# bdsaglam/torch-scae

Measured on AMD Instinct MI355X. Metric: images/sec SCAE fwd+bwd, MNIST 40x40 bs=128, 1/2/4/8 MI355X, higher is better.
Workload: dtype f32

## Files before the change

### include/scae_hip.h

```cpp
#ifndef SCAE_HIP_H
#define SCAE_HIP_H

#include <stdint.h>

#ifdef __cplusplus
extern "C" {
#endif

#define SCAE_ABI_VERSION 3

#define SCAE_OK 0
#define SCAE_ERR_BAD_ARG (-1)
#define SCAE_ERR_UNSUPPORTED (-2)

#define SCAE_MAX_CHANNELS 4
#define SCAE_ATTN_MAX_SET 64
#define SCAE_RENDER_MAX_TEMPLATE_ELEMS 4096

int scae_abi_version(void);
const char *scae_error_string(int code);

void *scae_launch_list_begin(void *stream);
int scae_launch_list_end(void *list);
int scae_launch_list_size(const void *list);
// ... 607 lines not shown
    const float *cls_b, const int64_t *label, const scae_loss_extras *extras, float *out12,
    float *workspace, int B, int O, int M, int ncls, int n_classes_cfg, int prior_type,
    int post_type, int sparsity_on, const float *weights5, float within_const,
    const float *cp_caps_presence, const float *cp_posterior, const float *cp_w,
    const float *cp_bias, float *prior_prob, float *post_prob, int cp_B, int cp_O, int cp_M,
    int cp_ncls, const scae_scaled_sum *extra_sums, int n_extra, void *stream);
int scae_loss_tail_fwd_class_probs_sink_f32(
    const float *lpp, const float *posterior, const float *caps_presence, const float *cls_w,
    const float *cls_b, const int64_t *label, const scae_loss_extras *extras, float *out12,
    float *workspace, int B, int O, int M, int ncls, int n_classes_cfg, int prior_type,
    int post_type, int sparsity_on, const float *weights5, float within_const,
    const float *cp_caps_presence, const float *cp_posterior, const float *cp_w,
    const float *cp_bias, float *prior_prob, float *post_prob, int cp_B, int cp_O, int cp_M,
    int cp_ncls, const scae_scaled_sum *extra_sums, int n_extra, scae_eval_sink *sink,
    void *stream);
int scae_loss_tail_bwd_f32(const float *lpp, const float *posterior,
                           const float *caps_presence, const float *cls_w,
                           const float *cls_b, const int64_t *label,
                           const scae_loss_extras *extras, const float *gout12,
                           const float *workspace, float *g_lpp, float *g_posterior,
                           float *g_caps_presence, float *g_cls_w,
                           float *g_cls_b, int B, int O, int M, int ncls, int n_classes_cfg,
                           int prior_type, int post_type, int sparsity_on,
                           const float *weights5, float within_const, void *stream);

#define SCAE_EVAL_ACC_DOUBLES 17
int scae_eval_tail_f32(const float *lpp, const float *posterior, const float *caps_presence,
                       const float *cls_w, const float *cls_b, const int64_t *label,
                       const scae_loss_extras *extras, float *out12, float *workspace, int B,
                       int O, int M, int ncls, int n_classes_cfg, int prior_type,
// ... 146 lines not shown
```

### torch_scae_amd/_lib.py

```python
import ctypes
import os
from ctypes import (POINTER, Structure, c_char_p, c_double, c_float, c_int,
                    c_int64, c_uint32, c_uint64, c_void_p)

_HERE = os.path.dirname(os.path.abspath(__file__))
LIB_PATH = os.environ.get("SCAE_HIP_LIB") or os.path.join(_HERE, "lib",
                                                        "libscae_hip.so")

P = c_void_p


class DecoderDesc(Structure):
    _fields_ = [("templates", P), ("templates_alpha", P), ("pose", P),
                ("presence", P), ("bg_image", P), ("bg_value", P),
                ("bg_mixing_logit", P), ("temperature_logit", P),
                ("out_scale", P),
                ("B", c_int), ("M", c_int), ("C", c_int), ("th", c_int),
                ("tw", c_int), ("H", c_int), ("W", c_int),
                ("template_repeat", c_int)]


class LikelihoodBwdDesc(Structure):
    _fields_ = [(n, P) for n in (
        "vote", "scale", "vote_presence", "dummy_vote", "x", "presence",
# ... 286 lines not shown
                                  + [c_int] * 7 + [P],
    "scae_capsule_votes_bwd_f32": [P] * 8 + [c_float] + [P] * 11
                                  + [c_int] * 7 + [P],
    "scae_capsule_likelihood_fwd_f32": [P] * 17 + [c_int] * 3 + [P],
    "scae_capsule_likelihood_bwd_f32": [P] * 22 + [c_int] * 3 + [P],
    "scae_loss_tail_supported": [c_int] * 3,
    "scae_loss_tail_workspace_floats": [c_int] * 3,
    "scae_loss_tail_fwd_f32": [P] * 6 + [POINTER(LossExtras), P, P] + [c_int] * 8
    + [POINTER(c_float), c_float, P],
    "scae_loss_tail_defer_preferred": [c_int] * 2,
    "scae_loss_tail_combine_f32": [P] * 6 + [POINTER(LossExtras), P, P] + [c_int] * 8
    + [POINTER(c_float), c_float, P],
    "scae_loss_tail_fwd_class_probs_f32": [P] * 6 + [POINTER(LossExtras), P, P]
    + [c_int] * 8 + [POINTER(c_float), c_float] + [P] * 6 + [c_int] * 4
    + [POINTER(ScaledSum), c_int, P],
    "scae_loss_tail_bwd_f32": [P] * 6 + [POINTER(LossExtras)] + [P] * 7
    + [c_int] * 8 + [POINTER(c_float), c_float, P],
    "scae_eval_tail_f32": [P] * 6 + [POINTER(LossExtras), P, P] + [c_int] * 8
    + [POINTER(c_float), c_float] + [P] * 5,
    "scae_loss_tail_fwd_class_probs_sink_f32": [P] * 6 + [POINTER(LossExtras), P, P]
    + [c_int] * 8 + [POINTER(c_float), c_float] + [P] * 6 + [c_int] * 4
    + [POINTER(ScaledSum), c_int, P, P],
    "scae_eval_tail_sink_f32": [P] * 6 + [POINTER(LossExtras), P, P] + [c_int] * 8
    + [POINTER(c_float), c_float] + [P] * 6,
    "scae_eval_accumulate_f32": [P] * 5 + [c_int] * 2 + [P] * 3,
    "scae_train_log_f32": [P] * 3 + [POINTER(TrainLogDesc), c_int, P],
    "scae_eval_features_f32": [P, P, c_int, c_int, c_int, P, P],
    "scae_kmeans_supported": [c_int] * 2,
    "scae_kmeans_groups": [c_int64, c_int],
    "scae_kmeans_lloyd_f32": [POINTER(KMeansDesc), c_int, P],
# ... 121 lines not shown
```

### torch_scae_amd/csrc/capsule_likelihood_dev.h

```cpp
#pragma once
#include "common.h"

namespace scae_lk {
namespace {
constexpr int NT = 1024;
constexpr int OMAX = 64;
constexpr float kLog001 = -4.605170185988091f;

__device__ __forceinline__ float vote_lp(const float *vt, const float *xv, float sc) {
  const float inv2v = 1.f / (2.f * sc * sc), ls = logf(sc);
  float acc = 0.f;
#pragma unroll
  for (int i = 0; i < 6; ++i) {
    const float d = xv[i] - vt[i];
    acc += -(d * d) * inv2v - ls - scae::kHalfLog2Pi;
  }
  return acc;
}

template <int G>
__device__ __forceinline__ float group_sum(float v) {
  static_assert(G == 16, "one DPP row");
  return scae::row_sum16(v);
}
// ... 103 lines not shown
      }
    }
    sm = group_sum<16>(sm);
    sp = group_sum<16>(sp);
    if (m < M && l == 0) {
      s.max_ml[m] = mx_ml;
      s.lse_ml[m] = mx_ml + logf(sm);
      s.max_post[m] = mx_po;
      s.sum_post[m] = sp;
      s.win[m] = (float)win;
    }
  }
  __syncthreads();
}

template <bool BIG>
__global__ __launch_bounds__(1024) void likelihood_fwd_kernel(
    LkArgs a, float *__restrict__ lpp, float *__restrict__ binary, float *__restrict__ winner,
    float *__restrict__ winner_presence, int64_t *__restrict__ winner_idx,
    int64_t *__restrict__ is_from_capsule, float *__restrict__ soft_winner,
    float *__restrict__ soft_winner_presence, float *__restrict__ posterior,
    float *__restrict__ mixing_log_prob, float *__restrict__ mixing_logit) {
  extern __shared__ __attribute__((aligned(16))) float smem[];
  const int O = a.O, M = a.M, tid = threadIdx.x;
  const LkSmem s = lk_carve(smem, O, M);
  for (int b = blockIdx.x; b < a.B; b += gridDim.x) {
    __syncthreads();
    lk_stats<BIG, NT>(a, s, b);
    for (int e = tid; e < (O + 1) * M; e += NT) {
      const int o = e / M, m = e - o * M;
      const size_t g1 = (size_t)b * (O + 1) * M + e;
      const float ml = o < O ? s.ml[e] : kLog001;
      const float post = o < O ? s.post[e] : kLog001 + kLog001;
      const float pp = expf(post - s.max_post[m]) / s.sum_post[m];
      mixing_logit[g1] = ml;
      mixing_log_prob[g1] = ml - s.lse_ml[m];
      posterior[g1] = pp;
      if (o < O) {
        binary[(size_t)b * O * M + e] = ml > kLog001 ? 1.f : 0.f;
        s.ml[e] = pp;
      }
    }
    __syncthreads();
    for (int t = tid; t < ((M * 7 * 4 + NT - 1) / NT) * NT; t += NT) {
      const int e = t >> 2, part = t & 3;
      const bool pose = e < M * 6, live = e < M * 7;
      const int m = pose ? e / 6 : e - M * 6, i = pose ? e - m * 6 : 0;
      float acc = 0.f;
      if (live) {
        if (pose) {
#pragma unroll 6
          for (int o = part; o < O; o += 4)
            acc = fmaf(s.ml[o * M + m], a.vote[(((size_t)b * O + o) * M + m) * 6 + i], acc);
        } else {
#pragma unroll 6
          for (int o = part; o < O; o += 4)
            acc = fmaf(s.ml[o * M + m], a.vp[((size_t)b * O + o) * M + m], acc);
        }
      }
      acc += scae::xor1_f(acc);
      acc += scae::xor2_f(acc);
      if (!live || part != 0) continue;
      const size_t idx = (size_t)b * M + m;
      const int win = (int)s.win[m];
      if (pose) {
        const float ppd = expf(kLog001 + kLog001 - s.max_post[m]) / s.sum_post[m];
        soft_winner[idx * 6 + i] = fmaf(ppd, a.dummy_vote[m * 6 + i], acc);
        winner[idx * 6 + i] = a.vote[(((size_t)b * O + win) * M + m) * 6 + i];
      } else {
        const float lse_post = s.max_post[m] + logf(s.sum_post[m]);
        lpp[idx] = a.presence ? lse_post * a.presence[idx] : lse_post;
        soft_winner_presence[idx] = acc;
        winner_presence[idx] = a.vp[((size_t)b * O + win) * M + m];
        winner_idx[idx] = win;
        is_from_capsule[idx] = win / M;
      }
    }
  }
}

template <bool BIG, int NT>
__device__ __forceinline__ void likelihood_bwd_body(
    LkArgs a, const int64_t *__restrict__ winner_idx, const float *__restrict__ g_lpp,
    const float *__restrict__ g_winner, const float *__restrict__ g_winner_presence,
    const float *__restrict__ g_soft_winner, const float *__restrict__ g_soft_winner_presence,
    const float *__restrict__ g_posterior, const float *__restrict__ g_mlp,
    const float *__restrict__ g_mlogit, float *__restrict__ gvote, float *__restrict__ gscale,
    float *__restrict__ gvp, float *__restrict__ gx, float *__restrict__ gpresence,
    float *__restrict__ gdummy, float *smem, int blk, int nblk) {
  const int O = a.O, M = a.M, tid = threadIdx.x;
  const LkSmem s = lk_carve(smem, O, M);
  float *s_gpp = s.aux;
// ... 124 lines not shown
```

### torch_scae_amd/csrc/loss_tail.hip

```cpp
#include "class_probs_dev.h"
#include "common.h"
#include "loss_tail_dev.h"

namespace {
using namespace scae_tail;
constexpr int MAXCLS = 32;

__device__ __forceinline__ float ent_term_grad(float p, float k) {
  const float q = p * k;
  return q < scae::kLogSafeEps ? 1e8f : -(logf(q) + 1.f);
}

__device__ __forceinline__ float within_term(const float *x, float r, int O, int type,
                                             float cw, int lane) {
  if (type == 0) return (r - cw) * (r - cw);
  const float k = type == 2 ? (float)O : 1.f;
  float w = 0.f;
  for (int o = lane; o < O; o += NTI) w += ent_term(x[o] / (r + 1e-8f), k);
  return scae::wave_sum(w);
}

__device__ __forceinline__ float cls_xe(const TailArgs &a, const float *x, int label, int lane,
                                        float &gl) {
  const bool on = lane < a.ncls;
// ... 11 lines not shown
    z = (z0 + z1) + (z2 + z3);
  }
  const float mx = scae::wave_max(z);
  float p = on ? expf(z - mx) : 0.f;
  p /= scae::wave_sum(p);
  const float mx2 = scae::wave_max(on ? p : -INFINITY);
  const float q = on ? expf(p - mx2) : 0.f;
  const float sum2 = scae::wave_sum(q);
  const float plabel = scae::wave_sum(lane == label ? p : 0.f);
  const float dq = on ? q / sum2 - (lane == label ? 1.f : 0.f) : 0.f;
  const float dot = scae::wave_sum(p * dq);
  gl = p * (dq - dot);
  return mx2 + logf(sum2) - plabel;
}

__global__ __launch_bounds__(NTI) void tail_image_kernel(TailArgs a, Ws ws, scae_cp::Args cpa,
                                                        int n_cp) {
  extern __shared__ __attribute__((aligned(16))) float smem[];
  const int B = a.B, O = a.O, M = a.M, b = blockIdx.x, lane = threadIdx.x;
  if (b >= B) {
    __shared__ scae_cp::Lds s_cpl;
    scae_cp::body(cpa, s_cpl, b - B, lane);
    return;
  }
  float *s_cp = smem, *s_mass = smem + O, *s_raw = smem + 2 * O;
  float rc = 0.f, rm = 0.f;
  for (int o = lane; o < O; o += NTI) {
    const float xc = a.cp[(size_t)b * O + o];
    const float *pr = a.posterior + ((size_t)b * (O + 1) + o) * M;
    float t = 0.f;
    if ((M & 3) == 0) {
      const float4 *p4 = reinterpret_cast<const float4 *>(pr);
      for (int m = 0; m < M / 4; ++m) {
        const float4 v = p4[m];
        t += (v.x + v.y) + (v.z + v.w);
      }
    } else {
      for (int m = 0; m < M; ++m) t += pr[m];
    }
// ... 18 lines not shown
  float xe_c = 0.f, xe_m = 0.f;
  if (a.label) {
    const int label = (int)a.label[b];
    float g0, g1;
    xe_c = cls_xe(a, s_cp, label, lane, g0);
    xe_m = cls_xe(a, s_raw, label, lane, g1);
    if (lane < a.ncls) {
      ws.gl[((size_t)b * 2 + 0) * a.ncls + lane] = g0;
      ws.gl[((size_t)b * 2 + 1) * a.ncls + lane] = g1;
    }
  }
  if (lane == 0) {
    float *p = ws.part + (size_t)b * 8;
    p[0] = lp, p[1] = wc, p[2] = wm, p[3] = xe_c, p[4] = xe_m, p[5] = rc, p[6] = rm, p[7] = 0.f;
  }
}

template <int NTC>
__global__ __launch_bounds__(NTC) void tail_combine_kernel(TailArgs a, scae_loss_extras x, Ws ws,
                                                          float *out) {
  extern __shared__ __attribute__((aligned(16))) float smem[];
  combine_body<NTC>(a, x, ws, out, smem);
}

template <int NTC>
__global__ __launch_bounds__(NTC) void tail_combine_log_kernel(TailArgs a, scae_loss_extras x,
                                                              Ws ws, float *out,
                                                              TrainLogArgs g) {
  extern __shared__ __attribute__((aligned(16))) float smem[];
  combine_body<NTC>(a, x, ws, out, smem);
// ... 300 lines not shown
extern "C" int scae_loss_tail_fwd_class_probs_f32(
    const float *lpp, const float *posterior, const float *caps_presence, const float *cls_w,
    const float *cls_b, const int64_t *label, const scae_loss_extras *extras, float *out12,
    float *workspace, int B, int O, int M, int ncls, int n_classes_cfg, int prior_type,
    int post_type, int sparsity_on, const float *weights5, float within_const,
    const float *cp_caps_presence, const float *cp_posterior, const float *cp_w,
    const float *cp_bias, float *prior_prob, float *post_prob, int cp_B, int cp_O, int cp_M,
    int cp_ncls, const scae_scaled_sum *extra_sums, int n_extra, void *stream) {
  return scae_loss_tail_fwd_class_probs_sink_f32(
      lpp, posterior, caps_presence, cls_w, cls_b, label, extras, out12, workspace, B, O, M,
      ncls, n_classes_cfg, prior_type, post_type, sparsity_on, weights5, within_const,
      cp_caps_presence, cp_posterior, cp_w, cp_bias, prior_prob, post_prob, cp_B, cp_O, cp_M,
      cp_ncls, extra_sums, n_extra, nullptr, stream);
}

extern "C" int scae_loss_tail_bwd_f32(const float *lpp, const float *posterior,
                                      const float *caps_presence, const float *cls_w,
                                      const float *cls_b, const int64_t *label,
                                      const scae_loss_extras *extras, const float *gout12,
                                      const float *workspace, float *g_lpp, float *g_posterior,
                                      float *g_caps_presence, float *g_cls_w, float *g_cls_b,
                                      int B, int O, int M, int ncls, int n_classes_cfg,
                                      int prior_type, int post_type, int sparsity_on,
                                      const float *weights5, float within_const, void *stream) {
  TailArgs a;
  int rc = fill_tail(a, lpp, posterior, caps_presence, cls_w, cls_b, label, B, O, M, ncls,
                     n_classes_cfg, prior_type, post_type, sparsity_on, weights5, within_const);
  if (rc) return rc;
  SCAE_REQUIRE(g_lpp && g_posterior && g_caps_presence && workspace);
  if (!gout12 && !(extras && extras->g_loss)) return SCAE_ERR_BAD_ARG;
// ... 33 lines not shown
```

### torch_scae_amd/object_decoder.py

```python
import torch
import torch.nn as nn

from . import math_ops, ops
from .general_utils import AttrDict, prod
from .nn_ext import GroupedMLP
from .nn_utils import rand_like


class CapsuleLayer(nn.Module):

    n_transform_params = 6

    def __init__(self, n_caps, dim_feature, n_votes, dim_caps,
                 hidden_sizes=(128,), caps_dropout_rate=0.0,
                 learn_vote_scale=False, allow_deformations=True,
                 noise_type=None, noise_scale=0., similarity_transform=True):
        super().__init__()
        self.n_caps = n_caps
        self.dim_feature = dim_feature
        self.hidden_sizes = list(hidden_sizes)
        self.dim_caps = dim_caps
        self.caps_dropout_rate = caps_dropout_rate
        self.n_votes = n_votes
        self.learn_vote_scale = learn_vote_scale
# ... 130 lines not shown
        return AttrDict(vote=vote, scale=scale, vote_presence=vote_presence,
                        presence_logit_per_caps=logit_caps,
                        presence_logit_per_vote=logit_vote,
                        cpr_dynamic_reg_loss=reg)


class CapsuleLikelihood:

    def __init__(self, vote, scale, vote_presence, dummy_vote):
        self.n_caps = vote.shape[1]
        self.vote = vote
        self.scale = scale
        self.vote_presence = vote_presence
        self.dummy_vote = dummy_vote

    def __call__(self, x, presence=None, _extra_sums=(), _defer_sums=False):
        batch_size, n_input_points, dim_in = x.shape
        if dim_in != 6 or self.vote.shape[-1] != 6:
            raise ValueError("the capsule likelihood kernel is built for "
                             "6-dim poses")
        (lpp, binary, winner, winner_presence, _widx, is_from_capsule,
         soft_winner, soft_winner_presence, posterior, mixing_log_prob,
         mixing_logit, log_prob) = ops.capsule_likelihood(
            self.vote, self.scale, self.vote_presence, self.dummy_vote, x,
            presence.float() if presence is not None else None,
            defer_sum=True)
        sums = [(lpp.detach(), 1.0 / batch_size, log_prob.detach()),
                *_extra_sums]
        if not _defer_sums:
            ops.scaled_sums(sums)
        return AttrDict(
            **(dict(_pending_sums=sums) if _defer_sums else {}),
            _log_prob_per_point=lpp,
            _posterior_full=posterior,
            log_prob=log_prob,
            vote_presence_binary=binary,
            winner=winner,
            winner_presence=winner_presence,
            soft_winner=soft_winner,
            soft_winner_presence=soft_winner_presence,
            posterior_mixing_prob=posterior[:, :-1],
# ... 3 lines not shown
        )


class CapsuleObjectDecoder(nn.Module):
    def __init__(self, capsule_layer: CapsuleLayer):
        super().__init__()
        self.capsule_layer = capsule_layer
        self.dummy_vote = nn.Parameter(torch.zeros(
            1, 1, capsule_layer.n_votes, capsule_layer.n_transform_params))

    @property
    def n_obj_capsules(self):
        return self.capsule_layer.n_caps

    def forward(self, obj_encoding: torch.Tensor, part_pose: torch.Tensor,
                part_presence: torch.Tensor = None, _defer_sums=False):
        vote, scale, vote_presence, logit_caps, logit_vote, reg, \
            caps_presence, reg_partial = self.capsule_layer._votes(
                obj_encoding, defer_reg=True)
        res = AttrDict(vote=vote,
                       scale=scale, vote_presence=vote_presence,
                       presence_logit_per_caps=logit_caps,
                       presence_logit_per_vote=logit_vote,
                       cpr_dynamic_reg_loss=reg)
        res.caps_presence = caps_presence
        likelihood = CapsuleLikelihood(vote=res.vote, scale=res.scale,
                                       vote_presence=res.vote_presence,
                                       dummy_vote=self.dummy_vote)
        res.update(likelihood(part_pose, presence=part_presence, _extra_sums=[
            (reg_partial, 0.5 / obj_encoding.shape[0], reg.detach())],
            _defer_sums=_defer_sums))
        return res


def capsule_l2_loss(caps_presence, n_classes: int,
                    within_example_constant=None, **_ignored):
    n_examples, n_caps = caps_presence.shape
    row_target = n_caps / n_classes if within_example_constant is None \
        else within_example_constant
    col_target = n_examples / n_classes
    row_mass, col_mass = caps_presence.sum(1), caps_presence.sum(0)
    return ((row_mass - row_target).square().mean(),
            (col_mass - col_target).square().mean())


def _scaled_self_entropy(mass, dim, k):
# ... 21 lines not shown
```

### torch_scae_amd/ops.py

```python
import ctypes
import functools

import numpy as np
import torch

from . import _lib, step_plan
from ._lib import DecoderDesc, ScaeHipError
from .step_plan import StepPlan, current as _plan

__all__ = ["geometric_transform", "qkv_attention", "set_encoder", "grouped_mlp", "seed_attention", "seed_attention_supported", "seed_fold", "seed_fold_supported", "loss_tail", "loss_tail_scalar", "loss_tail_supported", "capsule_votes",
           "capsule_likelihood", "colored_templates", "template_color_supported", "attention_conv_pool", "attention_pool_supported", "capsule_head", "part_encoder", "conv_stack", "conv_stack_supported",
           "uniform", "reset_noise", "pack_params", "render_templates", "render_gmm_log_prob", "render_gmm_log_prob_sums",
           "gmm_log_prob", "gmm_mean", "gmm_mode", "render_gmm_mode", "image_sheet", "ScaeHipError"]


def _need_hip(*tensors):
    for t in tensors:
        if t is None:
            continue
        if not t.is_cuda:
            raise ScaeHipError(
                "torch_scae_amd ops run only on a HIP device (got a "
                f"{t.device} tensor); there is no CPU path.")
        if t.dtype != torch.float32:
# ... 1365 lines not shown
                 similarity=False):
    pose, presence, feature, twin, absence = _PartEncoder.apply(
        image, tuple(int(s) for s in strides), post_bias, att_weight, att_bias,
        noise_u, n_caps, noise_scale, similarity, *weights, *biases)
    if feature.shape[-1] == 0:
        feature = twin = None
    return pose, presence, feature, twin, absence


def attention_conv_pool(x, weight, bias, n_caps):
    return _AttentionConvPool.apply(x, weight, bias, n_caps)


class _PendingClassProbs:

    def __init__(self, args, keep, stream_ref):
        self.args, self.keep, self.ref = args, keep, stream_ref

    def launch_alone(self):
        _lib.call("scae_class_probs_f32", *self.args, _stream(self.ref))


class _PendingCombine:

    def __init__(self, tail_args, keep, loss_ptr, out_ptr, stream_ref):
        self.tail, self.keep, self.ref = tail_args, keep, stream_ref
        self.loss_ptr, self.out_ptr = loss_ptr, out_ptr

    def launch_alone(self):
        ex = self.keep[-1]
        ex.defer_combine = 0
        _lib.call("scae_loss_tail_combine_f32", *self.tail, _stream(self.ref))


def flush_pending_forward():
# ... 9 lines not shown
    @_fwd
    def forward(ctx, caps_presence, posterior, weight, bias, extra_sums):
        _need_hip(caps_presence, posterior, weight, bias)
        cp, post = caps_presence.detach().contiguous(), \
            posterior.detach().contiguous()
        weight, bias = weight.contiguous(), bias.contiguous()
        B, O1, M = post.shape
        ncls = weight.shape[0]
        prior = torch.empty(B, ncls, device=cp.device, dtype=cp.dtype)
        posterior_prob = torch.empty_like(prior)
        extra = list(extra_sums or ())
        args = (_p(cp), _p(post), _p(weight), _p(bias), _p(prior),
                _p(posterior_prob), B, O1 - 1, M, ncls, _sum_jobs(extra),
                len(extra))
        if ctx.plan.fused:
            ctx.plan.flush_scope("fusing")
            ctx.plan.park("class_probs", _PendingClassProbs(
                args, (cp, post, weight, bias, prior, posterior_prob, extra),
                cp))
        else:
            _lib.call("scae_class_probs_f32", *args, _stream(cp))
        ctx.save_for_backward(cp, post, weight, bias)
        ctx.set_materialize_grads(False)
        return prior, posterior_prob

    @_bwd
    def backward(ctx, g_prior, g_post):
        cp, post, weight, bias = ctx.saved_tensors
        with torch.enable_grad():
            w, b = weight.detach().requires_grad_(), bias.detach().requires_grad_()
            outs, gs = [], []
            for x, g in ((cp, g_prior), (post[:, :-1].sum(-1), g_post)):
                if g is not None:
                    outs.append(torch.softmax(
# ... 759 lines not shown


def capsule_votes(all_param, cpr_static, bias_cvr, bias_caps, bias_vote,
                  bias_scale, noise_caps=None, noise_vote=None, noise_scale=0.,
                  similarity=False, learn_vote_scale=True,
                  allow_deformations=True, param_is_relu=False,
                  defer_reg=False):
    return _CapsuleVotes.apply(all_param, cpr_static, bias_cvr, bias_caps,
                               bias_vote, bias_scale, noise_caps, noise_vote,
                               noise_scale, similarity, learn_vote_scale,
                               allow_deformations, param_is_relu, defer_reg)


class _CapsuleLikelihood(torch.autograd.Function):
    @_fwd
    def forward(ctx, vote, scale, vp, dummy_vote, x, presence, defer_sum):
        _need_hip(vote, scale, vp, dummy_vote, x, presence)
        vote, scale, vp, dummy_vote, x, presence = (
            _c(t) for t in (vote, scale, vp, dummy_vote, x, presence))
        B, O, M, _ = vote.shape
        dev, dt = vote.device, vote.dtype
        f = lambda *s: torch.empty(*s, device=dev, dtype=dt)
        lpp, binary = f(B, M), f(B, O, M)
        winner, winner_p = f(B, M, 6), f(B, M)
        widx = torch.empty(B, M, device=dev, dtype=torch.int64)
        from_caps = torch.empty(B, M, device=dev, dtype=torch.int64)
        soft, soft_p = f(B, M, 6), f(B, M)
        post, mlp, mlogit = f(B, O + 1, M), f(B, O + 1, M), f(B, O + 1, M)
        log_prob = torch.empty((), device=dev, dtype=dt)
        _lib.call("scae_capsule_likelihood_fwd_f32", _p(vote), _p(scale),
                  _p(vp), _p(dummy_vote), _p(x), _p(presence), _p(lpp),
                  _p(binary), _p(winner), _p(winner_p), _p(widx),
                  _p(from_caps), _p(soft), _p(soft_p), _p(post), _p(mlp),
                  _p(mlogit), B, O, M, _stream(vote))
        if not defer_sum:
            scaled_sums([(lpp, 1.0 / B, log_prob)])
        saved = [vote, scale, vp, dummy_vote, x, post, widx]
        if presence is not None:
            saved.append(presence)
        ctx.save_for_backward(*saved)
        ctx.has_presence = presence is not None
        ctx.dims = (B, O, M)
        ctx.dummy_shape = dummy_vote.shape
        ctx.mark_non_differentiable(binary, widx, from_caps)
        ctx.set_materialize_grads(False)
        return (lpp, binary, winner, winner_p, widx, from_caps, soft, soft_p,
                post, mlp, mlogit, log_prob)

    @_bwd
# ... 33 lines not shown
            k.B, k.O, k.M = B, O, M
            _lib.call("scae_render_gmm_sums_bwd_likelihood_f32",
                      ctypes.byref(pending.desc), *pending.ptrs,
                      ctypes.byref(k), _stream(vote))
        else:
            if pending is not None:
                pending.launch_alone()
            _lib.call("scae_capsule_likelihood_bwd_f32", _p(vote), _p(scale),
                      _p(vp), _p(dummy_vote), _p(x), _p(presence), _p(post),
                      _p(widx), *[_p(g) for g in gin], _p(gvote), _p(gscale),
                      _p(gvp), _p(gx), _p(gpres), _p(gdummy), B, O, M,
                      _stream(vote))
        g_dummy = None
        if g_w is not None or g_s is not None:
            g_dummy = _sum_rows(gdummy.view(B, -1), [ctx.dummy_shape])[0]
        return gvote, gscale, gvp, g_dummy, gx, gpres, None


def capsule_likelihood(vote, scale, vote_presence, dummy_vote, x,
                       presence=None, defer_sum=False):
    return _CapsuleLikelihood.apply(vote, scale, vote_presence, dummy_vote, x,
                                    presence, defer_sum)


_SPARSITY_TYPES = {"l2": 0, "entropy": 1, "kl": 2}


def loss_tail_supported(B, O, n_classes):
    return bool(_lib.load().scae_loss_tail_supported(B, O, n_classes or 0))


class _LossTail(torch.autograd.Function):
    @_fwd
    def forward(ctx, lpp, posterior, caps_presence, cls_w, cls_b, label,
                rec_sums, reg, cfg):
        _need_hip(lpp, posterior, caps_presence, cls_w, cls_b, rec_sums, reg)
        ctx.slots = (_slot(cls_w, ctx), _slot(cls_b, ctx))
# ... 24 lines not shown
            bool(_lib.load().scae_loss_tail_defer_preferred(B, O))
        ev = ctx.plan.evaluation if ctx.plan.fused and rec_sums is not None else None
        if ev is not None and label is not None and not ctx.plan.holds("class_probs"):
            ev = None
        defer = defer and ev is None
        tl = ctx.plan.train_log if ctx.plan.fused and rec_sums is not None and ev is None \
            else None
        if tl is not None and label is not None and not ctx.plan.holds("class_probs"):
            tl = None
        ex.defer_combine = int(defer or ev is not None)
        ws = torch.empty(_lib.load().scae_loss_tail_workspace_floats(
            ints[0], ints[1], ints[3]), device=lpp.device, dtype=lpp.dtype)
        tail = (_p(lpp), _p(posterior), _p(caps_presence), _p(cls_w), _p(cls_b),
                lab, ctypes.byref(ex), _p(out), _p(ws), *ints, w5, wc)
        parked = ctx.plan.take("class_probs")
        if tl is not None:
            probs = (None, None) if label is None else parked.keep[4:6]
            ex.train_log = ctypes.pointer(tl.fused_desc(*probs, label))
        if ev is not None and parked is not None and ev.sink is not None:
            ev.sink_written = True
            _lib.call("scae_loss_tail_fwd_class_probs_sink_f32", *tail, *parked.args,
                      ctypes.c_void_p(ev.sink.ptr), _stream(lpp))
        elif parked is not None:
            _lib.call("scae_loss_tail_fwd_class_probs_f32", *tail, *parked.args,
                      _stream(lpp))
        else:
            _lib.call("scae_loss_tail_fwd_f32", *tail, _stream(lpp))
        if ev is not None:
            probs = (None, None) if label is None else parked.keep[4:6]
            ev.fused_launch(tail, *probs, keep=(ws, both, ex, w5), stream_ref=lpp)
        ctx.save_for_backward(lpp, posterior, caps_presence, ws,
                              *([cls_w, cls_b, label] if label is not None
                                else []),
                              *([rec_sums] if rec_sums is not None else []),
# ... 636 lines not shown
```

### torch_scae_amd/stacked_capsule_auto_encoder.py

```python
import torch
import torch.nn as nn
import torch.nn.functional as F

from . import nn_utils, ops
from .general_utils import LazyAttrDict
from .object_decoder import sparsity_loss


class SCAE(nn.Module):

    def __init__(self, part_encoder, template_generator, part_decoder,
                 obj_encoder, obj_decoder, n_classes=None, vote_type='soft',
                 presence_type='enc', stop_grad_caps_input=True,
                 stop_grad_caps_target=True, recon_mse_weight=0,
                 part_caps_sparsity_weight=0., cpr_dynamic_reg_weight=0.,
                 caps_ll_weight=0., prior_sparsity_loss_type='l2',
                 prior_within_example_sparsity_weight=0.,
                 prior_between_example_sparsity_weight=0.,
                 prior_within_example_constant=None,
                 posterior_sparsity_loss_type='entropy',
                 posterior_within_example_sparsity_weight=0.,
                 posterior_between_example_sparsity_weight=0.,
                 reconstruct_alternatives=True):
        super().__init__()
# ... 99 lines not shown
            obj_encoding = obj_encoding.to(image.dtype)
        target_pose, target_presence = parts.pose, parts.presence
        if self.stop_grad_caps_target:
            target_pose = target_pose.detach()
            target_presence = target_presence.detach()
        live_pose, live_presence = parts.pose, parts.presence
        phase_cut = None
        if self.split_backward and self.stop_grad_caps_target and \
                torch.is_grad_enabled() and \
                self.vote_type == self.presence_type == 'enc':
            srcs = [obj_encoding, templates, live_pose, live_presence]
            leaves = [t.detach().requires_grad_(t.requires_grad) for t in srcs]
            obj_encoding, templates, live_pose, live_presence = leaves
            phase_cut = (srcs, leaves)
        fused_probs = self._fused_class_probs(obj_encoding)
        res = self.obj_decoder(obj_encoding, target_pose, target_presence,
                               **(dict(_defer_sums=True) if fused_probs else {}))
        pending = res.pop("_pending_sums", None)
        res.part_presence = live_presence
        if phase_cut is not None:
            res._phase_cut = phase_cut

        dec_pose = {'enc': live_pose, 'soft': res.soft_winner,
                    'hard': res.winner}[self.vote_type]
        dec_presence = {'enc': live_presence,
                        'soft': res.soft_winner_presence,
                        'hard': res.winner_presence}[self.presence_type]
        res.rec = self.part_decoder(templates=templates, pose=dec_pose,
                                    presence=dec_presence)

        if self.reconstruct_alternatives:
            with torch.no_grad():
# ... 203 lines not shown
```

### torch_scae_amd/step_plan.py

```python
import collections
import contextlib
import contextvars
import weakref

ANY = "*"
_LIVE = weakref.WeakSet()


class Ride:

    __slots__ = ("carriers", "readers", "scope", "abi", "what")

    def __init__(self, what, carriers, readers=(), scope="deferring", abi=""):
        self.what, self.carriers, self.readers = what, tuple(carriers), readers
        self.scope, self.abi = scope, abi


RIDES = collections.OrderedDict([
    ("tc_fwd", Ride(
        "the colour MLP's forward (K10)",
        carriers=("_PartEncoder.forward",), scope="offer",
        abi="scae_capsule_head_conv_fwd_tc_f32")),
    ("logprob_fwd", Ride(
        "the reconstruction likelihood's forward (K1)",
        carriers=("_SetEncoder.forward",), scope="offer",
        abi="scae_set_encoder_fwd_logprob_f32")),
    ("class_probs", Ride(
        "SCAE.forward's two classifier heads (one wave per image)",
        carriers=("_LossTail.forward",), scope="fusing",
        abi="scae_loss_tail_fwd_class_probs_f32")),
    ("combine", Ride(
        "the loss tail's batch combine (one workgroup)",
        carriers=("_LossTail.backward",), scope="fusing",
        abi="scae_loss_tail_bwd_f32 (scae_loss_extras.defer_combine)")),
    ("k1_bwd", Ride(
        "the reconstruction likelihood's backward (K1)",
        carriers=("_CapsuleLikelihood.backward",), readers=ANY,
        abi="scae_render_gmm_sums_bwd_likelihood_f32")),
    ("wgrads", Ride(
        "the capsule MLPs' four weight-gradient GEMMs",
        carriers=("_SeedAttention.backward",),
        abi="scae_seed_attention_mfma_bwd_gemm_f32")),
    ("tc_bwd", Ride(
        "the colour MLP's backward (K10)",
        carriers=("_PartEncoder.backward",),
        readers=("_CapsuleHead.backward",),
        abi="scae_capsule_head_bwd_tc_f32")),
    ("reduce", Ride(
        "the output attention's partial-row reduction",
# ... 12 lines not shown
        self.name = name
        self.target = None
        self.rider = None
        self.offers = {}
        self.parked = {}
        self.deferred = None
        self.sums_to_optimizer = False
        self.held_sums = []
        self.prologue = prologue
        self.bf16 = False
        self.noise = {}
        self.noise_salt = 0
        self.side_stream = None
        self.evaluation = None
        self.train_log = None

    @contextlib.contextmanager
    def active(self):
        token = _CURRENT.set(self)
        try:
            yield self
        finally:
            _CURRENT.reset(token)

    @property
    def fused(self):
        return self.target is not None

    @property
    def parking(self):
# ... 147 lines not shown
```

Measured before the change: 265,000.

## Fuse capsule likelihood forward with loss tail and class probs into one kernel

Parks the capsule likelihood forward launch and, when the loss tail runs, launches a single kernel that computes the per-image likelihood outputs and then runs the per-image loss tail and class-prob bodies in the same workgroup. Late scaled sums that read likelihood outputs are handled by the last block, found through an atomic ticket counter. This removes a kernel launch and a global round trip of lpp/posterior between kernels. In exchange the tail work now runs in 1024-thread blocks with only 64 active lanes, and the launch logic carries extra parking and ordering bookkeeping.

```diff
diff --git a/include/scae_hip.h b/include/scae_hip.h
--- a/include/scae_hip.h
+++ b/include/scae_hip.h
@@ -645,6 +645,18 @@
     const float *cp_bias, float *prior_prob, float *post_prob, int cp_B, int cp_O, int cp_M,
     int cp_ncls, const scae_scaled_sum *extra_sums, int n_extra, scae_eval_sink *sink,
     void *stream);
+int scae_capsule_likelihood_fwd_loss_tail_f32(
+    const float *vote, const float *scale, const float *vote_presence, const float *dummy_vote,
+    const float *x, const float *presence, float *log_prob_per_point,
+    float *vote_presence_binary, float *winner, float *winner_presence, int64_t *winner_idx,
+    int64_t *is_from_capsule, float *soft_winner, float *soft_winner_presence, float *posterior,
+    float *mixing_log_prob, float *mixing_logit, const float *caps_presence, const float *cls_w,
+    const float *cls_b, const int64_t *label, const scae_loss_extras *extras, float *out12,
+    float *workspace, int B, int O, int M, int ncls, int n_classes_cfg, int prior_type,
+    int post_type, int sparsity_on, const float *weights5, float within_const,
+    const float *cp_caps_presence, const float *cp_w, const float *cp_bias, float *prior_prob,
+    float *post_prob, int cp_ncls, const scae_scaled_sum *extra_sums, int n_extra,
+    uint32_t *ticket, void *stream);
 int scae_loss_tail_bwd_f32(const float *lpp, const float *posterior,
                            const float *caps_presence, const float *cls_w,
                            const float *cls_b, const int64_t *label,
diff --git a/torch_scae_amd/_lib.py b/torch_scae_amd/_lib.py
--- a/torch_scae_amd/_lib.py
+++ b/torch_scae_amd/_lib.py
@@ -324,6 +324,9 @@
     "scae_loss_tail_fwd_class_probs_f32": [P] * 6 + [POINTER(LossExtras), P, P]
     + [c_int] * 8 + [POINTER(c_float), c_float] + [P] * 6 + [c_int] * 4
     + [POINTER(ScaledSum), c_int, P],
+    "scae_capsule_likelihood_fwd_loss_tail_f32": [P] * 17 + [P] * 4
+    + [POINTER(LossExtras), P, P] + [c_int] * 8 + [POINTER(c_float), c_float]
+    + [P] * 5 + [c_int, POINTER(ScaledSum), c_int, P, P],
     "scae_loss_tail_bwd_f32": [P] * 6 + [POINTER(LossExtras)] + [P] * 7
     + [c_int] * 8 + [POINTER(c_float), c_float, P],
     "scae_eval_tail_f32": [P] * 6 + [POINTER(LossExtras), P, P] + [c_int] * 8
diff --git a/torch_scae_amd/csrc/capsule_likelihood_dev.h b/torch_scae_amd/csrc/capsule_likelihood_dev.h
--- a/torch_scae_amd/csrc/capsule_likelihood_dev.h
+++ b/torch_scae_amd/csrc/capsule_likelihood_dev.h
@@ -141,6 +141,67 @@
   __syncthreads();
 }
 
+template <bool BIG, int NT>
+__device__ __forceinline__ void likelihood_fwd_image(
+    const LkArgs &a, const LkSmem &s, int b, float *__restrict__ lpp, float *__restrict__ binary,
+    float *__restrict__ winner, float *__restrict__ winner_presence,
+    int64_t *__restrict__ winner_idx, int64_t *__restrict__ is_from_capsule,
+    float *__restrict__ soft_winner, float *__restrict__ soft_winner_presence,
+    float *__restrict__ posterior, float *__restrict__ mixing_log_prob,
+    float *__restrict__ mixing_logit) {
+  const int O = a.O, M = a.M, tid = threadIdx.x;
+  lk_stats<BIG, NT>(a, s, b);
+  for (int e = tid; e < (O + 1) * M; e += NT) {
+    const int o = e / M, m = e - o * M;
+    const size_t g1 = (size_t)b * (O + 1) * M + e;
+    const float ml = o < O ? s.ml[e] : kLog001;
+    const float post = o < O ? s.post[e] : kLog001 + kLog001;
+    const float pp = expf(post - s.max_post[m]) / s.sum_post[m];
+    mixing_logit[g1] = ml;
+    mixing_log_prob[g1] = ml - s.lse_ml[m];
+    posterior[g1] = pp;
+    if (o < O) {
+      binary[(size_t)b * O * M + e] = ml > kLog001 ? 1.f : 0.f;
+      s.ml[e] = pp;
+    }
+  }
+  __syncthreads();
+  for (int t = tid; t < ((M * 7 * 4 + NT - 1) / NT) * NT; t += NT) {
+    const int e = t >> 2, part = t & 3;
+    const bool pose = e < M * 6, live = e < M * 7;
+    const int m = pose ? e / 6 : e - M * 6, i = pose ? e - m * 6 : 0;
+    float acc = 0.f;
+    if (live) {
+      if (pose) {
+#pragma unroll 6
+        for (int o = part; o < O; o += 4)
+          acc = fmaf(s.ml[o * M + m], a.vote[(((size_t)b * O + o) * M + m) * 6 + i], acc);
+      } else {
+#pragma unroll 6
+        for (int o = part; o < O; o += 4)
+          acc = fmaf(s.ml[o * M + m], a.vp[((size_t)b * O + o) * M + m], acc);
+      }
+    }
+    acc += scae::xor1_f(acc);
+    acc += scae::xor2_f(acc);
+    if (!live || part != 0) continue;
+    const size_t idx = (size_t)b * M + m;
+    const int win = (int)s.win[m];
+    if (pose) {
+      const float ppd = expf(kLog001 + kLog001 - s.max_post[m]) / s.sum_post[m];
+      soft_winner[idx * 6 + i] = fmaf(ppd, a.dummy_vote[m * 6 + i], acc);
+      winner[idx * 6 + i] = a.vote[(((size_t)b * O + win) * M + m) * 6 + i];
+    } else {
+      const float lse_post = s.max_post[m] + logf(s.sum_post[m]);
+      lpp[idx] = a.presence ? lse_post * a.presence[idx] : lse_post;
+      soft_winner_presence[idx] = acc;
+      winner_presence[idx] = a.vp[((size_t)b * O + win) * M + m];
+      winner_idx[idx] = win;
+      is_from_capsule[idx] = win / M;
+    }
+  }
+}
+
 template <bool BIG>
 __global__ __launch_bounds__(1024) void likelihood_fwd_kernel(
     LkArgs a, float *__restrict__ lpp, float *__restrict__ binary, float *__restrict__ winner,
@@ -149,60 +210,12 @@
     float *__restrict__ soft_winner_presence, float *__restrict__ posterior,
     float *__restrict__ mixing_log_prob, float *__restrict__ mixing_logit) {
   extern __shared__ __attribute__((aligned(16))) float smem[];
-  const int O = a.O, M = a.M, tid = threadIdx.x;
-  const LkSmem s = lk_carve(smem, O, M);
+  const LkSmem s = lk_carve(smem, a.O, a.M);
   for (int b = blockIdx.x; b < a.B; b += gridDim.x) {
     __syncthreads();
-    lk_stats<BIG, NT>(a, s, b);
-    for (int e = tid; e < (O + 1) * M; e += NT) {
-      const int o = e / M, m = e - o * M;
-      const size_t g1 = (size_t)b * (O + 1) * M + e;
-      const float ml = o < O ? s.ml[e] : kLog001;
-      const float post = o < O ? s.post[e] : kLog001 + kLog001;
-      const float pp = expf(post - s.max_post[m]) / s.sum_post[m];
-      mixing_logit[g1] = ml;
-      mixing_log_prob[g1] = ml - s.lse_ml[m];
-      posterior[g1] = pp;
-      if (o < O) {
-        binary[(size_t)b * O * M + e] = ml > kLog001 ? 1.f : 0.f;
-        s.ml[e] = pp;
-      }
-    }
-    __syncthreads();
-    for (int t = tid; t < ((M * 7 * 4 + NT - 1) / NT) * NT; t += NT) {
-      const int e = t >> 2, part = t & 3;
-      const bool pose = e < M * 6, live = e < M * 7;
-      const int m = pose ? e / 6 : e - M * 6, i = pose ? e - m * 6 : 0;
-      float acc = 0.f;
-      if (live) {
-        if (pose) {
-#pragma unroll 6
-          for (int o = part; o < O; o += 4)
-            acc = fmaf(s.ml[o * M + m], a.vote[(((size_t)b * O + o) * M + m) * 6 + i], acc);
-        } else {
-#pragma unroll 6
-          for (int o = part; o < O; o += 4)
-            acc = fmaf(s.ml[o * M + m], a.vp[((size_t)b * O + o) * M + m], acc);
-        }
-      }
-      acc += scae::xor1_f(acc);
-      acc += scae::xor2_f(acc);
-      if (!live || part != 0) continue;
-      const size_t idx = (size_t)b * M + m;
-      const int win = (int)s.win[m];
-      if (pose) {
-        const float ppd = expf(kLog001 + kLog001 - s.max_post[m]) / s.sum_post[m];
-        soft_winner[idx * 6 + i] = fmaf(ppd, a.dummy_vote[m * 6 + i], acc);
-        winner[idx * 6 + i] = a.vote[(((size_t)b * O + win) * M + m) * 6 + i];
-      } else {
-        const float lse_post = s.max_post[m] + logf(s.sum_post[m]);
-        lpp[idx] = a.presence ? lse_post * a.presence[idx] : lse_post;
-        soft_winner_presence[idx] = acc;
-        winner_presence[idx] = a.vp[((size_t)b * O + win) * M + m];
-        winner_idx[idx] = win;
-        is_from_capsule[idx] = win / M;
-      }
-    }
+    likelihood_fwd_image<BIG, NT>(a, s, b, lpp, binary, winner, winner_presence, winner_idx,
+                                  is_from_capsule, soft_winner, soft_winner_presence, posterior,
+                                  mixing_log_prob, mixing_logit);
   }
 }
 
diff --git a/torch_scae_amd/csrc/loss_tail.hip b/torch_scae_amd/csrc/loss_tail.hip
--- a/torch_scae_amd/csrc/loss_tail.hip
+++ b/torch_scae_amd/csrc/loss_tail.hip
@@ -1,3 +1,4 @@
+#include "capsule_likelihood_dev.h"
 #include "class_probs_dev.h"
 #include "common.h"
 #include "loss_tail_dev.h"
@@ -49,15 +50,9 @@
   return mx2 + logf(sum2) - plabel;
 }
 
-__global__ __launch_bounds__(NTI) void tail_image_kernel(TailArgs a, Ws ws, scae_cp::Args cpa,
-                                                        int n_cp) {
-  extern __shared__ __attribute__((aligned(16))) float smem[];
-  const int B = a.B, O = a.O, M = a.M, b = blockIdx.x, lane = threadIdx.x;
-  if (b >= B) {
-    __shared__ scae_cp::Lds s_cpl;
-    scae_cp::body(cpa, s_cpl, b - B, lane);
-    return;
-  }
+__device__ __forceinline__ void tail_image_body(const TailArgs &a, const Ws &ws, int b, int lane,
+                                                float *smem) {
+  const int O = a.O, M = a.M;
   float *s_cp = smem, *s_mass = smem + O, *s_raw = smem + 2 * O;
   float rc = 0.f, rm = 0.f;
   for (int o = lane; o < O; o += NTI) {
@@ -106,6 +101,50 @@
     float *p = ws.part + (size_t)b * 8;
     p[0] = lp, p[1] = wc, p[2] = wm, p[3] = xe_c, p[4] = xe_m, p[5] = rc, p[6] = rm, p[7] = 0.f;
   }
+}
+
+__global__ __launch_bounds__(NTI) void tail_image_kernel(TailArgs a, Ws ws, scae_cp::Args cpa,
+                                                        int n_cp) {
+  extern __shared__ __attribute__((aligned(16))) float smem[];
+  const int b = blockIdx.x, lane = threadIdx.x;
+  if (b >= a.B) {
+    __shared__ scae_cp::Lds s_cpl;
+    scae_cp::body(cpa, s_cpl, b - a.B, lane);
+    return;
+  }
+  tail_image_body(a, ws, b, lane, smem);
+}
+
+template <bool BIG>
+__global__ __launch_bounds__(1024) void likelihood_tail_kernel(
+    scae_lk::LkArgs la, float *lpp, float *binary, float *winner, float *winner_presence,
+    int64_t *winner_idx, int64_t *is_from_capsule, float *soft_winner,
+    float *soft_winner_presence, float *posterior, float *mixing_log_prob, float *mixing_logit,
+    TailArgs a, Ws ws, scae_cp::Args cpa, int has_cp, int n_free, unsigned *ticket) {
+  extern __shared__ __attribute__((aligned(16))) float smem[];
+  __shared__ scae_cp::Lds s_cpl;
+  const int B = a.B, b = blockIdx.x, tid = threadIdx.x;
+  if (b >= B) {
+    if (tid < 64) scae_cp::body(cpa, s_cpl, cpa.B + (b - B), tid);
+    return;
+  }
+  scae_lk::likelihood_fwd_image<BIG, 1024>(
+      la, scae_lk::lk_carve(smem, la.O, la.M), b, lpp, binary, winner, winner_presence,
+      winner_idx, is_from_capsule, soft_winner, soft_winner_presence, posterior, mixing_log_prob,
+      mixing_logit);
+  __syncthreads();
+  if (tid >= 64) return;
+  tail_image_body(a, ws, b, tid, smem);
+  if (has_cp) scae_cp::body(cpa, s_cpl, b, tid);
+  if (n_free == cpa.extra.n) return;
+  unsigned last = 0;
+  if (tid == 0)
+    last = __hip_atomic_fetch_add(ticket, 1u, __ATOMIC_ACQ_REL, __HIP_MEMORY_SCOPE_AGENT) ==
+           (unsigned)(B - 1);
+  if (!__shfl(last, 0)) return;
+  __threadfence();
+  if (tid == 0) __hip_atomic_store(ticket, 0u, __ATOMIC_RELAXED, __HIP_MEMORY_SCOPE_AGENT);
+  for (int j = n_free; j < cpa.extra.n; ++j) scae_cp::body(cpa, s_cpl, cpa.B + j, tid);
 }
 
 template <int NTC>
@@ -436,6 +475,89 @@
       cp_ncls, extra_sums, n_extra, nullptr, stream);
 }
 
+extern "C" int scae_capsule_likelihood_fwd_loss_tail_f32(
+    const float *vote, const float *scale, const float *vote_presence, const float *dummy_vote,
+    const float *x, const float *presence, float *log_prob_per_point,
+    float *vote_presence_binary, float *winner, float *winner_presence, int64_t *winner_idx,
+    int64_t *is_from_capsule, float *soft_winner, float *soft_winner_presence, float *posterior,
+    float *mixing_log_prob, float *mixing_logit, const float *caps_presence, const float *cls_w,
+    const float *cls_b, const int64_t *label, const scae_loss_extras *extras, float *out12,
+    float *workspace, int B, int O, int M, int ncls, int n_classes_cfg, int prior_type,
+    int post_type, int sparsity_on, const float *weights5, float within_const,
+    const float *cp_caps_presence, const float *cp_w, const float *cp_bias, float *prior_prob,
+    float *post_prob, int cp_ncls, const scae_scaled_sum *extra_sums, int n_extra,
+    uint32_t *ticket, void *stream) {
+  SCAE_REQUIRE(vote && scale && vote_presence && dummy_vote && x);
+  SCAE_REQUIRE(log_prob_per_point && vote_presence_binary && winner && winner_presence &&
+               winner_idx && is_from_capsule && soft_winner && soft_winner_presence &&
+               posterior && mixing_log_prob && mixing_logit);
+  if (B <= 0 || O <= 0 || M <= 0) return SCAE_ERR_BAD_ARG;
+  const size_t lk = scae_lk::lk_lds(O, M, false);
+  if (scae_lk::lk_lds(O, M, true) > 160 * 1024) return SCAE_ERR_UNSUPPORTED;
+  TailArgs a;
+  int rc = fill_tail(a, log_prob_per_point, posterior, caps_presence, cls_w, cls_b, label, B, O,
+                     M, ncls, n_classes_cfg, prior_type, post_type, sparsity_on, weights5,
+                     within_const);
+  if (rc) return rc;
+  SCAE_REQUIRE(out12 && workspace);
+  scae_loss_extras ex{};
+  if (extras) ex = *extras;
+  if (ex.rec_sums && ex.n_rec <= 0) return SCAE_ERR_BAD_ARG;
+  const Ws ws = carve_ws(workspace, B, O, ncls);
+  scae_cp::Args cpa{};
+  int n_free = 0;
+  if (cp_w) {
+    const float *const outs[] = {log_prob_per_point, vote_presence_binary, winner,
+                                 winner_presence, soft_winner, soft_winner_presence, posterior,
+                                 mixing_log_prob, mixing_logit};
+    const size_t BM = (size_t)B * M, n_out[] = {BM, BM * O, BM * 6, BM, BM * 6, BM,
+                                                BM * (O + 1), BM * (O + 1), BM * (O + 1)};
+    SCAE_REQUIRE(n_extra >= 0 && n_extra <= 8 && (n_extra == 0 || extra_sums));
+    scae_scaled_sum order[8];
+    int n_late = 0;
+    for (int pass = 0; pass < 2; ++pass)
+      for (int i = 0; i < n_extra; ++i) {
+        bool late = false;
+        for (int k = 0; k < 9; ++k)
+          late = late || (extra_sums[i].src < outs[k] + n_out[k] &&
+                          outs[k] < extra_sums[i].src + extra_sums[i].n);
+        if (late == (pass == 1)) order[pass == 0 ? n_free++ : n_free + n_late++] = extra_sums[i];
+      }
+    rc = scae_cp::fill(cpa, cp_caps_presence, posterior, cp_w, cp_bias, prior_prob, post_prob,
+                       B, O, M, cp_ncls, order, n_extra);
+    if (rc) return rc;
+    if (n_late) SCAE_REQUIRE(ticket);
+  } else if (n_extra) {
+    return SCAE_ERR_BAD_ARG;
+  }
+  scae_lk::LkArgs la{vote, scale, vote_presence, dummy_vote, x, presence, B, O, M};
+  const size_t lds = lk > 3 * O * sizeof(float) ? lk : 3 * O * sizeof(float);
+  const bool big = O > scae_lk::OMAX;
+  const void *fn = big ? reinterpret_cast<const void *>(likelihood_tail_kernel<true>)
+                       : reinterpret_cast<const void *>(likelihood_tail_kernel<false>);
+  if (lds > 48 * 1024) {
+    hipError_t e = hipFuncSetAttribute(fn, hipFuncAttributeMaxDynamicSharedMemorySize, (int)lds);
+    if (e != hipSuccess) return (int)e;
+  }
+  hipStream_t st = (hipStream_t)stream;
+#define SCAE_LK_TAIL(BG)                                                                         \
+  scae::launch(likelihood_tail_kernel<BG>, dim3(B + n_free), dim3(1024), lds, st, la,            \
+               log_prob_per_point, vote_presence_binary, winner, winner_presence, winner_idx,    \
+               is_from_capsule, soft_winner, soft_winner_presence, posterior, mixing_log_prob,   \
+               mixing_logit, a, ws, cpa, cp_w ? 1 : 0, n_free, ticket)
+  if (big) {
+    SCAE_LK_TAIL(true);
+  } else {
+    SCAE_LK_TAIL(false);
+  }
+#undef SCAE_LK_TAIL
+  if (!ex.defer_combine) {
+    rc = launch_combine(a, ex, ws, out12, st);
+    if (rc) return rc;
+  }
+  return scae_launch_status();
+}
+
 extern "C" int scae_loss_tail_bwd_f32(const float *lpp, const float *posterior,
                                       const float *caps_presence, const float *cls_w,
                                       const float *cls_b, const int64_t *label,
diff --git a/torch_scae_amd/object_decoder.py b/torch_scae_amd/object_decoder.py
--- a/torch_scae_amd/object_decoder.py
+++ b/torch_scae_amd/object_decoder.py
@@ -168,7 +168,8 @@
         self.vote_presence = vote_presence
         self.dummy_vote = dummy_vote
 
-    def __call__(self, x, presence=None, _extra_sums=(), _defer_sums=False):
+    def __call__(self, x, presence=None, _extra_sums=(), _defer_sums=False,
+                 _park=False):
         batch_size, n_input_points, dim_in = x.shape
         if dim_in != 6 or self.vote.shape[-1] != 6:
             raise ValueError("the capsule likelihood kernel is built for "
@@ -178,7 +179,7 @@
          mixing_logit, log_prob) = ops.capsule_likelihood(
             self.vote, self.scale, self.vote_presence, self.dummy_vote, x,
             presence.float() if presence is not None else None,
-            defer_sum=True)
+            defer_sum=True, park=_park and _defer_sums)
         sums = [(lpp.detach(), 1.0 / batch_size, log_prob.detach()),
                 *_extra_sums]
         if not _defer_sums:
@@ -212,7 +213,8 @@
         return self.capsule_layer.n_caps
 
     def forward(self, obj_encoding: torch.Tensor, part_pose: torch.Tensor,
-                part_presence: torch.Tensor = None, _defer_sums=False):
+                part_presence: torch.Tensor = None, _defer_sums=False,
+                _park=False):
         vote, scale, vote_presence, logit_caps, logit_vote, reg, \
             caps_presence, reg_partial = self.capsule_layer._votes(
                 obj_encoding, defer_reg=True)
@@ -227,7 +229,7 @@
                                        dummy_vote=self.dummy_vote)
         res.update(likelihood(part_pose, presence=part_presence, _extra_sums=[
             (reg_partial, 0.5 / obj_encoding.shape[0], reg.detach())],
-            _defer_sums=_defer_sums))
+            _defer_sums=_defer_sums, _park=_park))
         return res
 
 
diff --git a/torch_scae_amd/ops.py b/torch_scae_amd/ops.py
--- a/torch_scae_amd/ops.py
+++ b/torch_scae_amd/ops.py
@@ -1403,11 +1403,24 @@
 
 class _PendingClassProbs:
 
-    def __init__(self, args, keep, stream_ref):
+    def __init__(self, args, keep, stream_ref, plan):
         self.args, self.keep, self.ref = args, keep, stream_ref
+        self.plan = plan
 
     def launch_alone(self):
+        self.plan.flush("lk_fwd")
         _lib.call("scae_class_probs_f32", *self.args, _stream(self.ref))
+
+
+class _PendingLikelihood:
+
+    def __init__(self, ptrs, dims, keep, lpp, post):
+        self.ptrs, self.dims, self.keep = ptrs, dims, keep
+        self.lpp, self.post = lpp, post
+
+    def launch_alone(self):
+        _lib.call("scae_capsule_likelihood_fwd_f32", *self.ptrs, *self.dims,
+                  _stream(self.lpp))
 
 
 class _PendingCombine:
@@ -1447,10 +1460,10 @@
                 _p(posterior_prob), B, O1 - 1, M, ncls, _sum_jobs(extra),
                 len(extra))
         if ctx.plan.fused:
-            ctx.plan.flush_scope("fusing")
+            ctx.plan.flush("class_probs", "combine")
             ctx.plan.park("class_probs", _PendingClassProbs(
                 args, (cp, post, weight, bias, prior, posterior_prob, extra),
-                cp))
+                cp, ctx.plan))
         else:
             _lib.call("scae_class_probs_f32", *args, _stream(cp))
         ctx.save_for_backward(cp, post, weight, bias)
@@ -2240,7 +2253,8 @@
 
 class _CapsuleLikelihood(torch.autograd.Function):
     @_fwd
-    def forward(ctx, vote, scale, vp, dummy_vote, x, presence, defer_sum):
+    def forward(ctx, vote, scale, vp, dummy_vote, x, presence, defer_sum,
+                park):
         _need_hip(vote, scale, vp, dummy_vote, x, presence)
         vote, scale, vp, dummy_vote, x, presence = (
             _c(t) for t in (vote, scale, vp, dummy_vote, x, presence))
@@ -2254,11 +2268,19 @@
         soft, soft_p = f(B, M, 6), f(B, M)
         post, mlp, mlogit = f(B, O + 1, M), f(B, O + 1, M), f(B, O + 1, M)
         log_prob = torch.empty((), device=dev, dtype=dt)
-        _lib.call("scae_capsule_likelihood_fwd_f32", _p(vote), _p(scale),
-                  _p(vp), _p(dummy_vote), _p(x), _p(presence), _p(lpp),
-                  _p(binary), _p(winner), _p(winner_p), _p(widx),
-                  _p(from_caps), _p(soft), _p(soft_p), _p(post), _p(mlp),
-                  _p(mlogit), B, O, M, _stream(vote))
+        ptrs = (_p(vote), _p(scale), _p(vp), _p(dummy_vote), _p(x),
+                _p(presence), _p(lpp), _p(binary), _p(winner), _p(winner_p),
+                _p(widx), _p(from_caps), _p(soft), _p(soft_p), _p(post),
+                _p(mlp), _p(mlogit))
+        if park and defer_sum and ctx.plan.fused and \
+                ctx.plan.share_likelihood:
+            ctx.plan.park("lk_fwd", _PendingLikelihood(
+                ptrs, (B, O, M), (vote, scale, vp, dummy_vote, x, presence,
+                                  binary, winner, winner_p, widx, from_caps,
+                                  soft, soft_p, mlp, mlogit), lpp, post))
+        else:
+            _lib.call("scae_capsule_likelihood_fwd_f32", *ptrs, B, O, M,
+                      _stream(vote))
         if not defer_sum:
             scaled_sums([(lpp, 1.0 / B, log_prob)])
         saved = [vote, scale, vp, dummy_vote, x, post, widx]
@@ -2322,13 +2344,13 @@
         g_dummy = None
         if g_w is not None or g_s is not None:
             g_dummy = _sum_rows(gdummy.view(B, -1), [ctx.dummy_shape])[0]
-        return gvote, gscale, gvp, g_dummy, gx, gpres, None
+        return gvote, gscale, gvp, g_dummy, gx, gpres, None, None
 
 
 def capsule_likelihood(vote, scale, vote_presence, dummy_vote, x,
-                       presence=None, defer_sum=False):
+                       presence=None, defer_sum=False, park=False):
     return _CapsuleLikelihood.apply(vote, scale, vote_presence, dummy_vote, x,
-                                    presence, defer_sum)
+                                    presence, defer_sum, park)
 
 
 _SPARSITY_TYPES = {"l2": 0, "entropy": 1, "kl": 2}
@@ -2383,10 +2405,26 @@
         tail = (_p(lpp), _p(posterior), _p(caps_presence), _p(cls_w), _p(cls_b),
                 lab, ctypes.byref(ex), _p(out), _p(ws), *ints, w5, wc)
         parked = ctx.plan.take("class_probs")
+        lk = ctx.plan.take("lk_fwd")
+        if lk is not None and not (
+                ev is None and lk.lpp.data_ptr() == lpp.data_ptr()
+                and lk.post.data_ptr() == posterior.data_ptr()
+                and lk.dims == (B, O, M)
+                and (parked is None
+                     or parked.keep[1].data_ptr() == posterior.data_ptr())):
+            lk.launch_alone()
+            lk = None
         if tl is not None:
             probs = (None, None) if label is None else parked.keep[4:6]
             ex.train_log = ctypes.pointer(tl.fused_desc(*probs, label))
-        if ev is not None and parked is not None and ev.sink is not None:
+        if lk is not None:
+            a = parked.args if parked is not None else None
+            cp = (None,) * 5 + (0, None, 0) if a is None else \
+                (a[0], a[2], a[3], a[4], a[5], a[9], a[10], a[11])
+            _lib.call("scae_capsule_likelihood_fwd_loss_tail_f32", *lk.ptrs,
+                      *tail[2:], *cp, _p(ctx.plan.ticket(lpp.device)),
+                      _stream(lpp))
+        elif ev is not None and parked is not None and ev.sink is not None:
             ev.sink_written = True
             _lib.call("scae_loss_tail_fwd_class_probs_sink_f32", *tail, *parked.args,
                       ctypes.c_void_p(ev.sink.ptr), _stream(lpp))
diff --git a/torch_scae_amd/stacked_capsule_auto_encoder.py b/torch_scae_amd/stacked_capsule_auto_encoder.py
--- a/torch_scae_amd/stacked_capsule_auto_encoder.py
+++ b/torch_scae_amd/stacked_capsule_auto_encoder.py
@@ -137,8 +137,13 @@
             obj_encoding, templates, live_pose, live_presence = leaves
             phase_cut = (srcs, leaves)
         fused_probs = self._fused_class_probs(obj_encoding)
+        park = fused_probs and torch.is_grad_enabled() \
+            and not ops.evaluating() \
+            and self.vote_type == self.presence_type == 'enc' \
+            and not self.reconstruct_alternatives
         res = self.obj_decoder(obj_encoding, target_pose, target_presence,
-                               **(dict(_defer_sums=True) if fused_probs else {}))
+                               **(dict(_defer_sums=True, _park=park)
+                                  if fused_probs else {}))
         pending = res.pop("_pending_sums", None)
         res.part_presence = live_presence
         if phase_cut is not None:
diff --git a/torch_scae_amd/step_plan.py b/torch_scae_amd/step_plan.py
--- a/torch_scae_amd/step_plan.py
+++ b/torch_scae_amd/step_plan.py
@@ -33,6 +33,10 @@
         "the loss tail's batch combine (one workgroup)",
         carriers=("_LossTail.backward",), scope="fusing",
         abi="scae_loss_tail_bwd_f32 (scae_loss_extras.defer_combine)")),
+    ("lk_fwd", Ride(
+        "the capsule likelihood's forward (K4), one workgroup per image",
+        carriers=("_LossTail.forward",),
+        scope="fusing", abi="scae_capsule_likelihood_fwd_loss_tail_f32")),
     ("k1_bwd", Ride(
         "the reconstruction likelihood's backward (K1)",
         carriers=("_CapsuleLikelihood.backward",), readers=ANY,
@@ -75,6 +79,16 @@
         self.side_stream = None
         self.evaluation = None
         self.train_log = None
+        self._tickets = {}
+        self.share_likelihood = True
+
+    def ticket(self, device):
+        import torch
+        t = self._tickets.get(device)
+        if t is None:
+            t = self._tickets[device] = torch.zeros(1, device=device,
+                                                    dtype=torch.int32)
+        return t
 
     @contextlib.contextmanager
     def active(self):
```

After: 263,800 (median of 2 runs). No clear change (-0.5%).
